# terryye/cuda_FlashAttention

Measured on AMD Instinct MI355X. Metric: FA2 fwd+bwd TFLOP/s at (B=4,H=16,N=8192,d=128); % MFMA peak, higher is better.
Workload: dtype bf16; 1 GPU; FA2 forward+backward bf16, (B=4,H=16,N=8192,d=128) per GPU, non-causal (BASELINE configs[2]); flops = 14 B H N^2 d; B=4, H=16, N=8192, d=128, parallelism=head-sharded replicas x1

## Files before the change

### cuda_flashattention_amd/csrc/fa2_bwd_fused.hip

```cpp
#include <cstdlib>
#include <cstring>
#include <type_traits>

#include "fa2_common.h"
#include "fa2_launch.h"

namespace fa2 {

#include "fa2_bwd_fused_body.inc"

typedef __attribute__((address_space(3))) void* fused_lptr_t;

#ifndef FA2_FUSED_DSKEY
#define FA2_FUSED_DSKEY(row) (((row) >> 1) & 7)
#endif

#ifndef FA2_FUSED_DIAG
#define FA2_FUSED_DIAG 0
#endif

template <int R>
__device__ __forceinline__ void fused_vset(uint32_t x)
{
    asm volatile("v_mov_b32 v%c1, %0" : : "v"(x), "i"(R) : "v255");
}

#define FA2_FUSED_CLOBBERS "memory", "vcc", "v255", FA2_ACC_CLOBBERS
#define FA2_FUSED_OPS [r0] "v"(roff[0]), [r1] "v"(roff[1]), [r2] "v"(roff[2]), [r3] "v"(roff[3]), [r4] "v"(roff[4]), [r5] "v"(roff[5]),  \
    [r6] "v"(roff[6]), [r7] "v"(roff[7]), [t0] "v"(toff[0]), [t1] "v"(toff[1]), [t2] "v"(toff[2]), [t3] "v"(toff[3]), [t4] "v"(toff[4]),   \
    [t5] "v"(toff[5]), [t6] "v"(toff[6]), [t7] "v"(toff[7]), [rc] "v"(rcv), [c2] "s"(c2)

struct FusedStep {
    __amdgpu_buffer_rsrc_t drs, lrs, qrs, grs, rcrs, ctl;
    uint32_t dso, lso, qso, rcso, pvo, mso;
    int need, pval;
};
#define FA2_FUSED_OPS64 [r0] "v"(roff[0]), [r1] "v"(roff[1]), [r2] "v"(roff[2]), [r3] "v"(roff[3]), [t0] "v"(toff[0]), [t1] "v"(toff[1]),    \
    [t2] "v"(toff[2]), [t3] "v"(toff[3]), [rc] "v"(rcv), [c2] "s"(c2)
template <int BUF, int PAR, int VMW, bool MASKED>
__device__ __forceinline__ void fused_cbody(const uint32_t (&roff)[4], const uint32_t (&toff)[4], uint32_t rcv, float c2, uint32_t dqv,
                                            uint32_t dvo, uint32_t rcvo, uint32_t mw, uint32_t mw2, int wv, const FusedStep& f, int& err,
                                            int lo0 = 0, int lo1 = 0)
{
#define FA2_FUSED_CASE(B, P)                                                                                                          \
    if constexpr (BUF == B && PAR == P && MASKED)                                                                                     \
        asm volatile(FA2_FUSED64_MBODY_B##B##_P##P                                                                                    \
                     : [err] "+s"(err)                                                                                                \
                     : FA2_FUSED_OPS64, [vm] "i"(VMW), [dqv] "v"(dqv), [drs] "s"(f.drs), [dso] "s"(f.dso), [lrs] "s"(f.lrs), [lso] "s"(f.lso), \
                       [mw] "s"(mw), [mw2] "s"(mw2), [qrs] "s"(f.qrs), [grs] "s"(f.grs), [rcrs] "s"(f.rcrs), [qso] "s"(f.qso),           \
                       [rcso] "s"(f.rcso), [dvo] "v"(dvo), [rcvo] "v"(rcvo), [wv] "s"(wv), [ctl] "s"(f.ctl), [pvo] "s"(f.pvo),           \
                       [mso] "s"(f.mso), [need] "s"(f.need), [pval] "s"(f.pval), [lo0] "v"(lo0), [lo1] "v"(lo1)                        \
                     : FA2_FUSED_CLOBBERS, "s12", "s13", "scc", "exec", "m0", "v39");                                                 \
    if constexpr (BUF == B && PAR == P && !MASKED)                                                                                    \
        asm volatile(FA2_FUSED64_CBODY_B##B##_P##P                                                                                    \
                     : [err] "+s"(err)                                                                                                \
                     : FA2_FUSED_OPS64, [vm] "i"(VMW), [dqv] "v"(dqv), [drs] "s"(f.drs), [dso] "s"(f.dso), [lrs] "s"(f.lrs), [lso] "s"(f.lso), \
                       [mw] "s"(mw), [mw2] "s"(mw2), [qrs] "s"(f.qrs), [grs] "s"(f.grs), [rcrs] "s"(f.rcrs), [qso] "s"(f.qso),           \
                       [rcso] "s"(f.rcso), [dvo] "v"(dvo), [rcvo] "v"(rcvo), [wv] "s"(wv), [ctl] "s"(f.ctl), [pvo] "s"(f.pvo),           \
                       [mso] "s"(f.mso), [need] "s"(f.need), [pval] "s"(f.pval)                                                        \
                     : FA2_FUSED_CLOBBERS, "s12", "s13", "scc", "exec", "m0", "v39");
    FA2_FUSED_CASE(0, 0) FA2_FUSED_CASE(0, 1) FA2_FUSED_CASE(1, 0) FA2_FUSED_CASE(1, 1) FA2_FUSED_CASE(2, 0) FA2_FUSED_CASE(2, 1)
#undef FA2_FUSED_CASE
}

template <int BUF, int PAR, int VMW, bool MASKED>
__device__ __forceinline__ void fused_cbody(const uint32_t (&roff)[8], const uint32_t (&toff)[8], uint32_t rcv, float c2, uint32_t dqv,
                                            uint32_t dvo, uint32_t rcvo, uint32_t mw, uint32_t mw2, int wv, const FusedStep& f, int& err,
                                            int lo0 = 0, int lo1 = 0)
{
#define FA2_FUSED_CASE(B, P)                                                                                                          \
    if constexpr (BUF == B && PAR == P && MASKED)                                                                                     \
        asm volatile(FA2_FUSED_MBODY_B##B##_P##P                                                                                      \
                     : [err] "+s"(err)                                                                                                \
                     : FA2_FUSED_OPS, [vm] "i"(VMW), [dqv] "v"(dqv), [drs] "s"(f.drs), [dso] "s"(f.dso), [lrs] "s"(f.lrs), [lso] "s"(f.lso), \
                       [mw] "s"(mw), [mw2] "s"(mw2), [qrs] "s"(f.qrs), [grs] "s"(f.grs), [rcrs] "s"(f.rcrs), [qso] "s"(f.qso),           \
                       [rcso] "s"(f.rcso), [dvo] "v"(dvo), [rcvo] "v"(rcvo), [wv] "s"(wv), [ctl] "s"(f.ctl), [pvo] "s"(f.pvo),           \
                       [mso] "s"(f.mso), [need] "s"(f.need), [pval] "s"(f.pval), [lo0] "v"(lo0), [lo1] "v"(lo1)                        \
                     : FA2_FUSED_CLOBBERS, "s12", "s13", "scc", "exec", "m0", "v39");                                                 \
    if constexpr (BUF == B && PAR == P && !MASKED)                                                                                    \
        asm volatile(FA2_FUSED_CBODY_B##B##_P##P                                                                                      \
                     : [err] "+s"(err)                                                                                                \
                     : FA2_FUSED_OPS, [vm] "i"(VMW), [dqv] "v"(dqv), [drs] "s"(f.drs), [dso] "s"(f.dso), [lrs] "s"(f.lrs), [lso] "s"(f.lso), \
                       [mw] "s"(mw), [mw2] "s"(mw2), [qrs] "s"(f.qrs), [grs] "s"(f.grs), [rcrs] "s"(f.rcrs), [qso] "s"(f.qso),           \
                       [rcso] "s"(f.rcso), [dvo] "v"(dvo), [rcvo] "v"(rcvo), [wv] "s"(wv), [ctl] "s"(f.ctl), [pvo] "s"(f.pvo),           \
                       [mso] "s"(f.mso), [need] "s"(f.need), [pval] "s"(f.pval)                                                        \
                     : FA2_FUSED_CLOBBERS, "s12", "s13", "scc", "exec", "m0", "v39");
    FA2_FUSED_CASE(0, 0) FA2_FUSED_CASE(0, 1) FA2_FUSED_CASE(1, 0) FA2_FUSED_CASE(1, 1) FA2_FUSED_CASE(2, 0) FA2_FUSED_CASE(2, 1)
#undef FA2_FUSED_CASE
}

template <int BUF, int PAR, int VMW>
__device__ __forceinline__ void fused_body(const uint32_t (&roff)[8], const uint32_t (&toff)[8], uint32_t rcv, float c2)
{
#define FA2_FUSED_CASE(B, P) \
    if constexpr (BUF == B && PAR == P) asm volatile(FA2_FUSED_BODY_B##B##_P##P : : FA2_FUSED_OPS, [vm] "i"(VMW) : FA2_FUSED_CLOBBERS);
    FA2_FUSED_CASE(0, 0) FA2_FUSED_CASE(0, 1) FA2_FUSED_CASE(1, 0) FA2_FUSED_CASE(1, 1) FA2_FUSED_CASE(2, 0) FA2_FUSED_CASE(2, 1)
#undef FA2_FUSED_CASE
}

template <int DQT>
__device__ __forceinline__ void fused_dq_atomic(__amdgpu_buffer_rsrc_t rs, uint32_t voff, uint32_t soff)
{
    asm volatile(
        "s_add_u32 s12, %2, 4096\n\ts_add_u32 s13, %2, 8192\n\ts_add_u32 s14, %2, 12288\n\t"
        "buffer_atomic_add_f32 v%c3, %0, %1, %2 offen\n\tbuffer_atomic_add_f32 v%c4, %0, %1, %2 offen offset:512\n\t"
        "buffer_atomic_add_f32 v%c5, %0, %1, %2 offen offset:1024\n\tbuffer_atomic_add_f32 v%c6, %0, %1, %2 offen offset:1536\n\t"
        "buffer_atomic_add_f32 v%c7, %0, %1, s12 offen\n\tbuffer_atomic_add_f32 v%c8, %0, %1, s12 offen offset:512\n\t"
        "buffer_atomic_add_f32 v%c9, %0, %1, s12 offen offset:1024\n\tbuffer_atomic_add_f32 v%c10, %0, %1, s12 offen offset:1536\n\t"
        "buffer_atomic_add_f32 v%c11, %0, %1, s13 offen\n\tbuffer_atomic_add_f32 v%c12, %0, %1, s13 offen offset:512\n\t"
        "buffer_atomic_add_f32 v%c13, %0, %1, s13 offen offset:1024\n\tbuffer_atomic_add_f32 v%c14, %0, %1, s13 offen offset:1536\n\t"
        "buffer_atomic_add_f32 v%c15, %0, %1, s14 offen\n\tbuffer_atomic_add_f32 v%c16, %0, %1, s14 offen offset:512\n\t"
        "buffer_atomic_add_f32 v%c17, %0, %1, s14 offen offset:1024\n\tbuffer_atomic_add_f32 v%c18, %0, %1, s14 offen offset:1536\n\t"
        "s_nop 1"
        : : "v"(voff), "s"(rs), "s"(soff), "i"(DQT), "i"(DQT + 1), "i"(DQT + 2), "i"(DQT + 3), "i"(DQT + 4), "i"(DQT + 5), "i"(DQT + 6),
            "i"(DQT + 7), "i"(DQT + 8), "i"(DQT + 9), "i"(DQT + 10), "i"(DQT + 11), "i"(DQT + 12), "i"(DQT + 13), "i"(DQT + 14),
            "i"(DQT + 15)
        : "memory", "s12", "s13", "s14", "v255");
}

template <int VF, int KS, int S>
__device__ __forceinline__ void fused_load_vfrag(const char* v0, const char* v1)
{
#ifndef FA2_FUSED_KV_NT
#define FA2_FUSED_KV_NT ""
#define FA2_FUSED_KV_AUX 0
#endif
    asm volatile("global_load_dwordx4 v[%c2:%c3], %0, off offset:%c4" FA2_FUSED_KV_NT "\n\tglobal_load_dwordx4 v[%c5:%c6], %1, off offset:%c4" FA2_FUSED_KV_NT
                 : : "v"(v0), "v"(v1), "i"(VF + 4 * S), "i"(VF + 4 * S + 3), "i"(32 * S), "i"(VF + 4 * (KS + S)), "i"(VF + 4 * (KS + S) + 3)
                 : "memory", "v255");
}

template <int T>
__device__ __forceinline__ void fused_acc_zero(u32x4 z)
{
    asm volatile("s_nop 1\n\tv_mfma_f32_32x32x16_bf16 a[%c1:%c2], %0, %0, 0" : : "v"(z), "i"(16 * T), "i"(16 * T + 15) : FA2_ACC_CLOBBERS);
}

template <int DQT>
__device__ __forceinline__ void fused_dq_zero()
{
    static_for<16>([&](auto R) { fused_vset<DQT + decltype(R)::value>(0u); });
}

constexpr int kCtlTicket = 0, kCtlNextHead = 32 * 16, kCtlError = 32 * 17, kCtlHeadmap = 32 * 18;
constexpr int kHmPad = 16;
constexpr int kSpinLimit = FA2_FUSED_SPIN_LIMIT;

struct FusedArgs {
    BwdArgs b;
    float* dQacc;
    int* ctl;
    int npad;
    const float* rc;
    int fault;
};

#ifdef FA2_TEST_HOOKS
static int g_hook_fault = 0, g_hook_grid = 0, g_hook_last_grid = 0;
extern "C" void fa2_test_set_fused_hooks(int fault, int grid) { g_hook_fault = fault; g_hook_grid = grid; }
extern "C" int fa2_test_last_fused_grid(void) { return g_hook_last_grid; }
#define FA2_HOOK_NOTE_GRID(n) (g_hook_last_grid = (n))
#else
constexpr int g_hook_fault = 0, g_hook_grid = 0;
#define FA2_HOOK_NOTE_GRID(n) ((void)0)
#endif

__device__ __forceinline__ int fused_ctl_ints(int BH, int ncb) { return kCtlHeadmap + 16 * (BH + kHmPad) + 9 * BH * ncb; }

__device__ __forceinline__ int fused_load_sc1(const int* p)
{
    int v;
    asm volatile("global_load_dword %0, %1, off sc1\n\ts_waitcnt vmcnt(0)" : "=v"(v) : "v"(p) : "memory");
    return v;
}
__device__ __forceinline__ void fused_seen_set(int v)
{
    asm volatile("v_mov_b32 v39, %0" : : "s"(v) : "v39");
}

__device__ __forceinline__ int fused_lane_id() { return (int)__builtin_amdgcn_mbcnt_hi(~0u, __builtin_amdgcn_mbcnt_lo(~0u, 0u)); }
template <int OFF>
__device__ __forceinline__ int fused_mail_read(uint32_t lds_addr)
{
    int v;
    asm volatile("v_mov_b32 %0, %1\n\tds_read_b32 %0, %0 offset:%c2\n\ts_waitcnt lgkmcnt(0)" : "=&v"(v) : "s"(lds_addr), "i"(OFF) : "memory");
    return __builtin_amdgcn_readfirstlane(v);
}

__device__ __forceinline__ void fused_store_flag(int* p, int v)
{
    asm volatile("global_store_dword %0, %1, off" : : "v"(p), "v"(v) : "memory");
}

__device__ __forceinline__ bool fused_spin_over(int* ctl, int spins)
{
    if (spins > kSpinLimit) {
        atomicExch(ctl + kCtlError, 1);
        return true;
    }
    return (spins & 1023) == 0 && fused_load_sc1(ctl + kCtlError) != 0;
}

template <bool CHAIN, bool CAUSAL, bool RAGGED = false, bool RECT = false, int HD = 128>
__global__ void __launch_bounds__(256, 1) __attribute__((amdgpu_num_vgpr(39))) fa2_bwd_fused_kernel(FusedArgs fp)
{
    static_assert(CHAIN || !RAGGED, "the atomics form has no ragged variant");
    static_assert(!RECT || (CHAIN && !CAUSAL && !RAGGED), "rectangular blocks: chained, unmasked, aligned");
    static_assert(HD == 128 || (HD == 64 && CHAIN && !RECT), "head_dim 64: chained, square");
    extern __shared__ __attribute__((aligned(16))) char smem[];
    const BwdArgs& p = fp.b;
    constexpr int D = HD, ROWB = 2 * D, KS = D / 16, DT = D / 32;
    constexpr int DQW = 128;
    constexpr int TROWS = 32;
    constexpr bool W = D == 128;
    constexpr int QRING = W ? FA2_FUSED_QRING : FA2_FUSED64_QRING, BUFB = W ? FA2_FUSED_BUFB : FA2_FUSED64_BUFB,
                  DSB = W ? FA2_FUSED_DSB : FA2_FUSED64_DSB, LDSB = W ? FA2_FUSED_LDS : FA2_FUSED64_LDS;
    constexpr int CPR = D / 8, RPI = 64 / CPR, NINS = TROWS / RPI;
    constexpr int VF = W ? FA2_FUSED_VF : FA2_FUSED64_VF, DQT = W ? FA2_FUSED_DQT : FA2_FUSED64_DQT,
                  ROFFK = W ? FA2_FUSED_ROFFK : FA2_FUSED64_ROFFK, DSWR = W ? FA2_FUSED_DSWR : FA2_FUSED64_DSWR,
                  DSRD = W ? FA2_FUSED_DSRD : FA2_FUSED64_DSRD, KT = W ? FA2_FUSED_KT : FA2_FUSED64_KT;
    constexpr int VMW = CHAIN ? (W ? 4 : 2) : 63;
    int* const mail = reinterpret_cast<int*>(smem + LDSB);
    const uint32_t mail_addr = __builtin_amdgcn_readfirstlane((uint32_t)(uintptr_t)smem) + LDSB;

    const int tid = threadIdx.x;
    const int lane = tid & 63;
    const int wave = __builtin_amdgcn_readfirstlane(tid >> 6);
    const int ki = lane & 31;
    const int h = lane >> 5;
    const int N = p.Nk;
    const int NP = RAGGED ? fp.npad : N;
    const int NQ = RECT ? p.Nq : N;
    const int NPQ = RECT ? NQ : NP;
    const int QHS = RECT ? p.q_hs : N, KHS = RECT ? p.k_hs : N;
    const int QR0 = RECT ? p.q_row0 : 0;
    const int ncb = NP / 256;
    const int ntiles = NPQ / TROWS;
    const int niter = ((ntiles + 1 + 5) / 6) * 6;
    const float c2 = p.scale * kLog2e;
    const size_t rc_plane = (size_t)p.BH * (RECT ? QHS : NP);

    const uint32_t lbase = (uint32_t)(uintptr_t)smem;
    const int trq = (lane & 15) >> 2, trp = lane & 3, trcb = (lane >> 4) & 1;
    uint32_t roff[KS], toff[2 * DT];
#pragma unroll
    for (int s = 0; s < KS; ++s) roff[s] = lbase + QRING + lds_off<D>(ki, 2 * s + h);
#pragma unroll
    for (int dt = 0; dt < DT; ++dt)
#pragma unroll
        for (int jj = 0; jj < 2; ++jj)
            toff[2 * dt + jj] = lbase + QRING + lds_off<D>(8 * jj + 4 * h + trq, 4 * dt + 2 * trcb + (trp >> 1)) + 8 * (trp & 1);
    const uint32_t rcv = lbase + QRING + 2 * TROWS * ROWB + 16 * h;
    static_for<KS>([&](auto S) {
        constexpr int sidx = decltype(S)::value;
        fused_vset<ROFFK + sidx>(lbase + lds_off<D>(ki + 64 * wave, 2 * sidx + h));
    });
    const int ecol = W ? wave : (wave & 1), ekey0 = W ? 0 : 128 * (wave >> 1);
    static_for<2>([&](auto JJ) {
        constexpr int jj = decltype(JJ)::value;
        fused_vset<KT + jj>(lbase + ekey0 * ROWB + lds_off<D>(8 * jj + 4 * h + trq, 4 * ecol + 2 * trcb + (trp >> 1)) + 8 * (trp & 1));
        const int row = 8 * jj + 4 * h + trq;
        fused_vset<DSRD + jj>(lbase + DSB + (ekey0 + row) * 64 + 8 * ((4 * trcb + trp) ^ FA2_FUSED_DSKEY(row)));
    });
    static_for<4>([&](auto C) {
        constexpr int c = decltype(C)::value;
        fused_vset<DSWR + c>(lbase + DSB + (64 * wave + ki) * 64 + 8 * (((2 * c) | h) ^ FA2_FUSED_DSKEY(ki)));
    });
    const int drow = lane / CPR, dslot = lane % CPR;
    const int prow = wave * RPI + drow;
    const int doff = drow * ROWB + 16 * ((lds_off<D>(prow, dslot) - ROWB * prow) >> 4);
    const uint32_t dqv = CHAIN ? (uint32_t)(wave * 4096 + lane * 16) : (uint32_t)(((4 * h) * D + 32 * wave + ki) * 4);
    const auto rc_rsrc = __builtin_amdgcn_make_buffer_rsrc((void*)fp.rc, 0, (int)(2 * rc_plane * 4), 0x00020000);

    int xcc = 0;
    if constexpr (CHAIN) {
        asm volatile("s_getreg_b32 %0, hwreg(HW_REG_XCC_ID, 0, 4)" : "=s"(xcc));
    }
    int* const prog_base = fp.ctl + kCtlHeadmap + 16 * (p.BH + kHmPad);
#ifndef FA2_FUSED_CAUSAL_G
#define FA2_FUSED_CAUSAL_G 2
#endif
    const int G = CAUSAL ? max(1, min(FA2_FUSED_CAUSAL_G, p.BH / 8)) : 1;
    const auto ctl_rsrc = __builtin_amdgcn_make_buffer_rsrc((void*)fp.ctl, 0, CHAIN ? fused_ctl_ints(p.BH, ncb) * 4 : 0, 0x00020000);

    auto take_ticket = [&]() {
        if (wave == 0 && fused_lane_id() == 0) {
            int hd, j = 0;
            do {
                const int u = atomicAdd(fp.ctl + kCtlTicket + 32 * xcc, 1);
                const int r = u % (G * ncb);
                const int k = (u / (G * ncb)) * G + r % G;
                j = r / G;
                hd = -2;
                if (k < p.BH + kHmPad) {
                    int* hm = fp.ctl + kCtlHeadmap + xcc * (p.BH + kHmPad) + k;
                    int v = 0, spins = 0;
                    if (j == 0) {
                        if (k > 0)
                            while ((v = fused_load_sc1(hm - 1)) == 0)
                                if (fused_spin_over(fp.ctl, ++spins)) break;
                        if (k > 0 && v == 0) {
                            v = -1;
                        } else {
                            const int g = atomicAdd(fp.ctl + kCtlNextHead, 1);
                            v = g < p.BH ? g + 1 : -1;
                        }
                        fused_store_flag(hm, v);
                    } else {
                        while ((v = fused_load_sc1(hm)) == 0)
                            if (fused_spin_over(fp.ctl, ++spins)) { v = -1; break; }
                    }
                    hd = v > 0 ? v - 1 : (r % G == 0 ? -2 : -1);
                }
            } while (hd == -1);
            mail[0] = hd;
            mail[1] = j;
            mail[2] = hd >= 0 ? fused_load_sc1(fp.ctl + kCtlError) : 0;
        }
    };
    auto issue_unit_loads = [&](int head_, int cb_) {
        const size_t slab_ = (size_t)(head_ / p.kv_group) * KHS * ROWB;
        const char* Kh_ = (const char*)p.K + slab_;
        const char* Vh_ = (const char*)p.V + slab_;
        const int kw0_ = cb_ * 256 + wave * 64;
        const int lane_u = (int)__builtin_amdgcn_mbcnt_hi(~0u, __builtin_amdgcn_mbcnt_lo(~0u, 0u));
        const int vk0 = RAGGED ? min(kw0_ + (lane_u & 31), N - 1) : kw0_ + (lane_u & 31);
        const int vk1 = RAGGED ? min(kw0_ + 32 + (lane_u & 31), N - 1) : kw0_ + 32 + (lane_u & 31);
        const char* v0 = Vh_ + (size_t)vk0 * ROWB + 16 * (lane_u >> 5);
        const char* v1 = Vh_ + (size_t)vk1 * ROWB + 16 * (lane_u >> 5);
        static_for<KS>([&](auto S) { fused_load_vfrag<VF, KS, decltype(S)::value>(v0, v1); });
        const auto k_rsrc = __builtin_amdgcn_make_buffer_rsrc((void*)Kh_, 0, N * ROWB, 0x00020000);
#pragma unroll
        for (int j = wave; j < 256 / RPI; j += 4)
            __builtin_amdgcn_raw_ptr_buffer_load_lds(k_rsrc, (fused_lptr_t)(smem + j * 1024), 16, doff, (cb_ * 256 + j * RPI) * ROWB, 0, FA2_FUSED_KV_AUX);
    };

    auto next_unit_loads = [&]() {
        if constexpr (CHAIN) {
            take_ticket();
            __syncthreads();
            const int hn = fused_mail_read<0>(mail_addr);
            if (hn >= 0) issue_unit_loads(hn, fused_mail_read<4>(mail_addr));
        }
    };
    next_unit_loads();

    for (;;) {
#ifdef FA2_FUSED_STATS
        const uint64_t s_pull = __builtin_readcyclecounter();
#endif
        int head, cb, err0 = 0;
        if constexpr (CHAIN) {
            head = fused_mail_read<0>(mail_addr);
            cb = fused_mail_read<4>(mail_addr);
            err0 = fused_mail_read<8>(mail_addr);
            if (head < 0) break;
        } else {
            map_block(blockIdx.x, p.BH, ncb, head, cb);
            issue_unit_loads(head, cb);
        }
        const size_t slab = (size_t)head * QHS * ROWB;
        const char* Qh = (const char*)p.Q + slab;
        const char* Gh = (const char*)p.dO + slab;
        const int kw0 = cb * 256 + wave * 64;
        {
            const u32x4 z = {0u, 0u, 0u, 0u};
            static_for<4 * DT>([&](auto T) { fused_acc_zero<decltype(T)::value>(z); });
        }

        const auto q_rsrc = __builtin_amdgcn_make_buffer_rsrc((void*)Qh, 0, NQ * ROWB, 0x00020000);
        const auto g_rsrc = __builtin_amdgcn_make_buffer_rsrc((void*)Gh, 0, NQ * ROWB, 0x00020000);
        const int rcoff = (int)(((wave == 0 ? 0 : rc_plane) + (size_t)head * (RECT ? QHS : NP) + QR0 + (fused_lane_id() & 31)) * 4);
        auto stage = [&](int t, int buf) {
            char* b = smem + QRING + buf * BUFB;
#pragma unroll
            for (int j = wave; j < 2 * NINS; j += 4) {
                const int which = j / NINS, piece = j % NINS;
                const int soff = (t * TROWS + piece * RPI) * ROWB;
                __builtin_amdgcn_raw_ptr_buffer_load_lds(which ? g_rsrc : q_rsrc, (fused_lptr_t)(b + which * (TROWS * ROWB) + piece * 1024),
                                                         16, doff, soff, 0, 0);
            }
            if (wave < 2 && fused_lane_id() < 32)
                __builtin_amdgcn_raw_ptr_buffer_load_lds(rc_rsrc, (fused_lptr_t)(b + 2 * TROWS * ROWB + wave * 128), 4, rcoff, t * TROWS * 4, 0, 0);
        };
        const int n_u = CAUSAL ? ntiles - 8 * cb : ntiles;
        const int niter_u = CAUSAL ? ((n_u + 1 + 5) / 6) * 6 : niter;
        const bool ragged_unit = RAGGED && !CAUSAL && cb == ncb - 1;
        const int first_masked = CAUSAL ? ((n_u - 8) / 6) * 6 : (ragged_unit ? 0 : niter_u);
        auto tl = [&](int u) { return CAUSAL ? ntiles - 1 - u : u; };
        stage(tl(0), 0);
#ifdef FA2_FUSED_PREFILL
        stage(tl(1), 1);
        stage(tl(2), 2);
#endif
        fused_dq_zero<DQT>();
        asm volatile("s_waitcnt vmcnt(0)" ::: "memory");
        __syncthreads();
        if constexpr (W) asm volatile(FA2_FUSED_PRO : : FA2_FUSED_OPS, [vm] "i"(VMW) : FA2_FUSED_CLOBBERS);
        else asm volatile(FA2_FUSED64_PRO : : FA2_FUSED_OPS64, [vm] "i"(VMW) : FA2_FUSED_CLOBBERS);

        const auto dq_rsrc = __builtin_amdgcn_make_buffer_rsrc((void*)(fp.dQacc + (size_t)head * NPQ * DQW), 0, NPQ * DQW * 4, 0x00020000);
        int* const mine = prog_base + head * ncb + cb;
        const int* const prev = mine - 1;
        const int prev_off = (int)((prev - fp.ctl) * 4);
        const int mine_off = (int)((mine - fp.ctl) * 4);
        if constexpr (CHAIN) fused_seen_set(0);
        int err = err0;
#ifdef FA2_FUSED_STATS
        int st_steps = 0, st_polls = 0, st_cycles = 0;
        const uint64_t u0 = __builtin_readcyclecounter();
#endif

        const auto null_rsrc = __builtin_amdgcn_make_buffer_rsrc((void*)fp.dQacc, 0, 0, 0x00020000);
        const bool hp_unit = cb > 0;
        const auto lrs_unit = hp_unit && !(FA2_FUSED_DIAG & 2) ? dq_rsrc : null_rsrc;
        auto step = [&](auto BUF, auto PAR, auto MASKED, auto FAST_, int t) {
            constexpr int buf = decltype(BUF)::value, par = decltype(PAR)::value;
            constexpr bool masked = decltype(MASKED)::value;
            constexpr bool FAST = decltype(FAST_)::value;
            if constexpr (CHAIN && FAST) {
                FusedStep f;
                f.drs = dq_rsrc;
                f.lrs = lrs_unit;
                f.dso = (uint32_t)(tl(t - 1) * TROWS * DQW * 4);
                f.lso = (uint32_t)(tl(t) * TROWS * DQW * 4);
                f.qrs = q_rsrc; f.grs = g_rsrc; f.rcrs = rc_rsrc; f.ctl = ctl_rsrc;
                f.qso = (uint32_t)(tl(t + 1) * TROWS * ROWB + wave * 1024);
                f.rcso = (uint32_t)(tl(t + 1) * TROWS * 4);
                f.pvo = (uint32_t)prev_off; f.mso = (uint32_t)mine_off;
                f.need = (hp_unit && !err && !(FA2_FUSED_DIAG & 1)) ? t + 1 : (int)0x80000000;
                f.pval = t;
#ifdef FA2_TEST_HOOKS
                if (fp.fault && cb == 1) f.pval = 0;
#endif
                fused_cbody<buf, par, VMW, false>(roff, toff, rcv, c2, dqv, (uint32_t)doff, (uint32_t)rcoff, lbase + QRING + wave * 1024,
                                                  lbase + QRING + wave * 128, wave, f, err, 0, 0);
            } else if constexpr (CHAIN) {
                FusedStep f;
                const bool live = t >= 1 && t <= n_u;
                const bool more = t + 1 < n_u;
                const bool has_prev = t < n_u && cb > 0;
                f.drs = live ? dq_rsrc : null_rsrc;
                f.lrs = has_prev && !(FA2_FUSED_DIAG & 2) ? dq_rsrc : null_rsrc;
                f.dso = (uint32_t)__builtin_amdgcn_readfirstlane(tl(t - 1) * TROWS * DQW * 4);
                f.lso = (uint32_t)__builtin_amdgcn_readfirstlane(tl(t) * TROWS * DQW * 4);
                f.qrs = q_rsrc; f.grs = g_rsrc; f.rcrs = rc_rsrc; f.ctl = ctl_rsrc;
                f.qso = more ? (uint32_t)(tl(t + 1) * TROWS * ROWB + wave * 1024) : 0x40000000u;
                f.rcso = more ? (uint32_t)(tl(t + 1) * TROWS * 4) : 0x40000000u;
                f.pvo = (uint32_t)prev_off; f.mso = (uint32_t)mine_off;
                f.need = (has_prev && !err && !(FA2_FUSED_DIAG & 1)) ? t + 1 : (int)0x80000000;
                f.pval = t < n_u ? t : n_u;
#ifdef FA2_TEST_HOOKS
                if (fp.fault && cb == 1) f.pval = 0;
#endif
                int lo0 = 0, lo1 = 0;
                if constexpr (masked) {
                    const int lane_m = (int)__builtin_amdgcn_mbcnt_hi(~0u, __builtin_amdgcn_mbcnt_lo(~0u, 0u));
                    if constexpr (CAUSAL) {
                        lo0 = kw0 + (lane_m & 31) - 4 * (lane_m >> 5) - TROWS * tl(t);
                        lo1 = lo0 + 32;
                    } else {
                        lo0 = kw0 + (lane_m & 31) < N ? -0x40000000 : 0x40000000;
                        lo1 = kw0 + 32 + (lane_m & 31) < N ? -0x40000000 : 0x40000000;
                    }
                }
#ifdef FA2_FUSED_STATS2
                const uint64_t b0 = __builtin_readcyclecounter();
#endif
                fused_cbody<buf, par, VMW, masked>(roff, toff, rcv, c2, dqv, (uint32_t)doff, (uint32_t)rcoff, lbase + QRING + wave * 1024,
                                                   lbase + QRING + wave * 128, wave, f, err, lo0, lo1);
#ifdef FA2_FUSED_STATS2
                st_cycles += (int)(__builtin_readcyclecounter() - b0);
#endif
            } else {
                static_assert(W || CHAIN, "head_dim 64: chained form only");
                stage(t + 1, (buf + 1) % 3);
                if constexpr (W) fused_body<buf, par, VMW>(roff, toff, rcv, c2);
#ifndef FA2_FUSED_NO_DQ
                if (t >= 1 && t <= ntiles) fused_dq_atomic<DQT>(dq_rsrc, dqv, (uint32_t)__builtin_amdgcn_readfirstlane((t - 1) * TROWS * D * 4));
#endif
                fused_dq_zero<DQT>();
            }
        };
        auto six = [&](auto MASKED, auto FAST_, int t) {
            step(std::integral_constant<int, 0>{}, std::integral_constant<int, 0>{}, MASKED, FAST_, t);
            step(std::integral_constant<int, 1>{}, std::integral_constant<int, 1>{}, MASKED, FAST_, t + 1);
            step(std::integral_constant<int, 2>{}, std::integral_constant<int, 0>{}, MASKED, FAST_, t + 2);
            step(std::integral_constant<int, 0>{}, std::integral_constant<int, 1>{}, MASKED, FAST_, t + 3);
            step(std::integral_constant<int, 1>{}, std::integral_constant<int, 0>{}, MASKED, FAST_, t + 4);
            step(std::integral_constant<int, 2>{}, std::integral_constant<int, 1>{}, MASKED, FAST_, t + 5);
        };
        const int fast_end = CHAIN ? n_u - 2 : -1;
        {
            const int plain_end = first_masked;
            int t = 0;
            asm volatile("" : "+s"(t));
            if (t < plain_end) { six(std::false_type{}, std::false_type{}, t); t += 6; }
#pragma unroll 1
            for (; t + 5 <= fast_end && t < plain_end; t += 6) six(std::false_type{}, std::true_type{}, t);
#pragma unroll 1
            for (; t < plain_end; t += 6) six(std::false_type{}, std::false_type{}, t);
            if constexpr (CHAIN && (CAUSAL || RAGGED)) {
#pragma unroll 1
                for (; t < niter_u; t += 6) six(std::true_type{}, std::false_type{}, t);
            }
        }
        asm volatile("s_waitcnt vmcnt(0) lgkmcnt(0)" ::: "memory");
        if constexpr (CHAIN)
            if (err && !err0 && wave == 0 && fused_lane_id() == 0) atomicExch(fp.ctl + kCtlError, 1);
#ifdef FA2_FUSED_STATS
        const uint64_t s_loop = __builtin_readcyclecounter();
#endif
        next_unit_loads();

        mfma_acc_settle();
        const int lane_ep = (int)__builtin_amdgcn_mbcnt_hi(~0u, __builtin_amdgcn_mbcnt_lo(~0u, 0u));
        const int ki_ep = lane_ep & 31, h_ep = lane_ep >> 5;
        static_for<2>([&](auto KB) {
            constexpr int kb = decltype(KB)::value;
            const int key = kw0 + 32 * kb + ki_ep;
            const size_t slab_k = RECT ? (size_t)head * KHS * ROWB : slab;
            char* const dKb = (char*)p.dK + slab_k;
            char* const dVb = (char*)p.dV + slab_k;
            const uint32_t koff = (uint32_t)key * ROWB + 16u * h_ep;
            char* dKk = dKb + koff;
            char* dVk = dVb + koff;
            static_for<2 * DT>([&](auto G) {
                constexpr int dt = decltype(G)::value / 2, gp = decltype(G)::value % 2;
                constexpr int RK = 16 * (kb * DT + dt) + 8 * gp, RV = 32 * DT + RK;
                auto pack4 = [&](float a, float b, float c, float d, float sc) {
                    bf16x4 v;
                    v[0] = (__bf16)(a * sc); v[1] = (__bf16)(b * sc); v[2] = (__bf16)(c * sc); v[3] = (__bf16)(d * sc);
                    return __builtin_bit_cast(u32x2, v);
                };
                auto emit = [&](u32x2 x, u32x2 y, char* dst) {
                    const auto s0 = __builtin_amdgcn_permlane32_swap(x[0], y[0], false, false);
                    const auto s1 = __builtin_amdgcn_permlane32_swap(x[1], y[1], false, false);
                    const u32x4 o = {s0[0], s1[0], s0[1], s1[1]};
#ifdef FA2_FUSED_ST_NT
                    if (!RAGGED || key < N) __builtin_nontemporal_store(o, reinterpret_cast<u32x4*>(dst + 2 * (32 * dt + 16 * gp)));
#else
                    if (!RAGGED || key < N) *reinterpret_cast<u32x4*>(dst + 2 * (32 * dt + 16 * gp)) = o;
#endif
                };
                emit(pack4(acc_read<RK>(), acc_read<RK + 1>(), acc_read<RK + 2>(), acc_read<RK + 3>(), p.scale),
                     pack4(acc_read<RK + 4>(), acc_read<RK + 5>(), acc_read<RK + 6>(), acc_read<RK + 7>(), p.scale), dKk);
                emit(pack4(acc_read<RV>(), acc_read<RV + 1>(), acc_read<RV + 2>(), acc_read<RV + 3>(), 1.0f),
                     pack4(acc_read<RV + 4>(), acc_read<RV + 5>(), acc_read<RV + 6>(), acc_read<RV + 7>(), 1.0f), dVk);
            });
        });
#ifdef FA2_FUSED_STATS
        if (CHAIN && wave == 0 && fused_lane_id() == 0) {
            atomicAdd(fp.ctl + kCtlError + 1, st_steps);
            atomicAdd(fp.ctl + kCtlError + 2, st_polls);
            atomicAdd((unsigned long long*)(fp.ctl + kCtlError + 4), (unsigned long long)st_cycles);
            atomicAdd((unsigned long long*)(fp.ctl + kCtlError + 6), (unsigned long long)(__builtin_readcyclecounter() - u0));
            int* rec = prog_base + p.BH * ncb + 8 * (head * ncb + cb);
            rec[0] = xcc; rec[1] = st_cycles; rec[2] = (int)(u0 - s_pull); rec[3] = (int)(__builtin_readcyclecounter() - s_loop);
            *(unsigned long long*)(rec + 4) = u0; *(unsigned long long*)(rec + 6) = __builtin_readcyclecounter();
        }
#endif
        if constexpr (!CHAIN) break;
    }
}

__global__ void __launch_bounds__(256) fa2_bwd_fused_dq_out_kernel(const float* __restrict__ acc, __bf16* __restrict__ dQ, size_t n8, float scale,
                                                                    const int* __restrict__ err)
{
    const float poison = (err && *err) ? __builtin_nanf("") : 0.0f;
    const size_t stride = (size_t)gridDim.x * 256;
    for (size_t i = (size_t)blockIdx.x * 256 + threadIdx.x; i < n8; i += stride) {
        const f32x4 a = reinterpret_cast<const f32x4*>(acc)[2 * i], b = reinterpret_cast<const f32x4*>(acc)[2 * i + 1];
        bf16x8 o;
#pragma unroll
        for (int e = 0; e < 4; ++e) { o[e] = (__bf16)(a[e] * scale + poison); o[4 + e] = (__bf16)(b[e] * scale + poison); }
        reinterpret_cast<bf16x8*>(dQ)[i] = o;
    }
}

__global__ void __launch_bounds__(256) fa2_bwd_fused_dq_out_chain_kernel(const float* __restrict__ acc, __bf16* __restrict__ dQ, size_t n4, float scale,
                                                                          const int* __restrict__ err, int N, int NP, int qhs)
{
    const float poison = *err ? __builtin_nanf("") : 0.0f;
    const size_t stride = (size_t)gridDim.x * 256;
    const size_t tiles = (size_t)(NP / 32);
    for (size_t i = (size_t)blockIdx.x * 256 + threadIdx.x; i < n4; i += stride) {
        const f32x4 a = reinterpret_cast<const f32x4*>(acc)[i];
        const int lane = (int)(i & 63), g = (int)((i >> 6) & 3), wave = (int)((i >> 8) & 3);
        const size_t tg = i >> 10, head = tg / tiles;
        const int row = (int)(tg % tiles) * 32 + 8 * g + 4 * (lane >> 5);
        __bf16* o = dQ + (head * (size_t)qhs + row) * 128 + 32 * wave + (lane & 31);
#pragma unroll
        for (int e = 0; e < 4; ++e)
            if (row + e < N) o[(size_t)e * 128] = (__bf16)(a[e] * scale + poison);
    }
}

__global__ void __launch_bounds__(256) fa2_bwd_fused_dq_out_chain64_kernel(const float* __restrict__ acc, __bf16* __restrict__ dQ, size_t n4h, float scale,
                                                                            const int* __restrict__ err, int N, int NP)
{
    const float poison = *err ? __builtin_nanf("") : 0.0f;
    const size_t stride = (size_t)gridDim.x * 256;
    const size_t tiles = (size_t)(NP / 32);
    for (size_t i = (size_t)blockIdx.x * 256 + threadIdx.x; i < n4h; i += stride) {
        const int lane = (int)(i & 63), g = (int)((i >> 6) & 3), cbk = (int)((i >> 8) & 1);
        const size_t tg = i >> 9, head = tg / tiles;
        const size_t slot = ((tg * 4 + cbk) * 4 + g) * 64 + lane;
        const f32x4 a = reinterpret_cast<const f32x4*>(acc)[slot], b = reinterpret_cast<const f32x4*>(acc)[slot + 2 * 4 * 64];
        const int row = (int)(tg % tiles) * 32 + 8 * g + 4 * (lane >> 5);
        __bf16* o = dQ + (head * (size_t)N + row) * 64 + 32 * cbk + (lane & 31);
#pragma unroll
        for (int e = 0; e < 4; ++e)
            if (row + e < N) o[(size_t)e * 64] = (__bf16)((a[e] + b[e]) * scale + poison);
    }
}

__global__ void __launch_bounds__(256) fa2_bwd_fused_dkdv_out_kernel(const bf16x8* __restrict__ pK, const bf16x8* __restrict__ pV,
                                                                      bf16x8* __restrict__ dK, bf16x8* __restrict__ dV, size_t n8, size_t nkv, int G)
{
    const size_t stride = (size_t)gridDim.x * 256;
    for (size_t i = (size_t)blockIdx.x * 256 + threadIdx.x; i < 2 * nkv * n8; i += stride) {
        const bool isv = i >= nkv * n8;
        const size_t o = isv ? i - nkv * n8 : i, kvh = o / n8, r = o % n8;
        const bf16x8* src = (isv ? pV : pK) + kvh * (size_t)G * n8 + r;
        float s[8] = {};
        for (int g = 0; g < G; ++g) {
            const bf16x8 x = src[(size_t)g * n8];
#pragma unroll
            for (int e = 0; e < 8; ++e) s[e] += (float)x[e];
        }
        bf16x8 out;
#pragma unroll
        for (int e = 0; e < 8; ++e) out[e] = (__bf16)s[e];
        (isv ? dV : dK)[o] = out;
    }
}

__global__ void __launch_bounds__(256) fa2_bwd_fused_rcpad_kernel(const float* __restrict__ rc, float* __restrict__ out, int BH, int N, int NP)
{
    const size_t per = (size_t)BH * NP, i = (size_t)blockIdx.x * 256 + threadIdx.x;
    if (i >= 2 * per) return;
    const size_t plane = i / per, r = i % per, head = r / NP;
    const int row = (int)(r % NP);
    out[i] = row < N ? rc[plane * (size_t)BH * N + head * (size_t)N + row] : (plane == 0 ? -1.0e30f : 0.0f);
}

bool bwd_fused_device_ok(const char** why)
{
    static int verdict[64] = {};
    int dev = 0;
    if (hipGetDevice(&dev) != hipSuccess || dev < 0 || dev >= 64) { if (why) *why = "no current device"; return false; }
    if (!verdict[dev]) {
        hipDeviceProp_t pr;
        if (hipGetDeviceProperties(&pr, dev) != hipSuccess) { if (why) *why = "device properties unavailable"; return false; }
        verdict[dev] = strncmp(pr.gcnArchName, "gfx950", 6) != 0 ? 2 : pr.multiProcessorCount != 256 ? 3 : 1;
    }
    static const char* const text[] = {"", "single five-product kernel (gfx950, 256 CUs: the layout the ordered hand-off was validated on)",
                                       "two kernels: device is not gfx950", "two kernels: device does not expose 256 CUs (partitioned GPU): "
                                       "the ordered hand-off was validated in SPX mode only"};
    if (why) *why = text[verdict[dev]];
    return verdict[dev] == 1;
}

hipError_t bwd_fused_read_error(const int* ctl, int* err, hipStream_t stream)
{
    hipError_t e = hipMemcpyAsync(err, ctl + kCtlError, sizeof(int), hipMemcpyDeviceToHost, stream);
    if (e != hipSuccess) return e;
    return hipStreamSynchronize(stream);
}

hipError_t bwd_fused_clear_error(int* ctl, hipStream_t stream)
{
    return launch_fill_f32(reinterpret_cast<float*>(ctl + kCtlError), 1, 0.0f, stream);
}

size_t bwd_fused_kvpart_bytes(int BH, int N, int d) { return (size_t)2 * BH * N * d * 2; }
size_t bwd_fused_ctl_bytes(int BH, int N) { return (size_t)(kCtlHeadmap + 16 * (BH + kHmPad) + 9 * BH * ((N + 255) / 256)) * sizeof(int); }

template <int HD>
static hipError_t launch_chained_square(bool causal, bool ragged, dim3 grid, int lds, hipStream_t stream, const FusedArgs& fa)
{
    if (causal)
        return ragged ? launch_lds<fa2_bwd_fused_kernel<true, true, true, false, HD>>(grid, dim3(256), lds, stream, fa)
                      : launch_lds<fa2_bwd_fused_kernel<true, true, false, false, HD>>(grid, dim3(256), lds, stream, fa);
    return ragged ? launch_lds<fa2_bwd_fused_kernel<true, false, true, false, HD>>(grid, dim3(256), lds, stream, fa)
                  : launch_lds<fa2_bwd_fused_kernel<true, false, false, false, HD>>(grid, dim3(256), lds, stream, fa);
}

hipError_t launch_bwd_fused_bf16(const BwdArgs& a, float* dQacc, int* ctl, int mode, hipStream_t stream, float* rcpad, void* kvpart)
{
    const int npad = (a.Nk + 255) / 256 * 256;
    const bool ragged = npad != a.Nk;
    const bool rect = a.Nq != a.Nk || a.q_hs != a.Nq || a.k_hs != a.Nk || a.q_row0 != 0;
    if ((a.d != 128 && a.d != 64) || a.Nk < 1 || a.Nq < 1) return hipErrorInvalidValue;
    if (a.d == 64 && (mode != 1 || rect)) return hipErrorInvalidValue;
    if (rect && (mode != 1 || a.causal || ragged || a.Nq % 32 != 0 || a.q_row0 < 0 || a.q_hs < a.q_row0 + a.Nq || a.k_hs < a.Nk))
        return hipErrorInvalidValue;
    if (ragged && (mode != 1 || !rcpad)) return hipErrorInvalidValue;
    const bool grouped = a.kv_group > 1;
    if (a.kv_group < 1 || a.BH % a.kv_group != 0 || (grouped && (mode != 1 || rect || !kvpart))) return hipErrorInvalidValue;
    if (a.causal && (mode != 1 || a.causal_shift != 0)) return hipErrorInvalidValue;
    hipError_t e = hipSuccess;
    if (a.phases & 1) {
        BwdArgs d = a;
        d.phases = 1;
        e = launch_bwd_bf16(d, stream);
        if (e != hipSuccess) return e;
    }
    if (!(a.phases & 8)) return hipSuccess;
    const size_t elems = (size_t)a.BH * (rect ? a.Nq : npad) * 128;
    const int units = a.BH * (npad / 256);
    if (ragged) {
        const size_t n = (size_t)2 * a.BH * npad;
        hipLaunchKernelGGL(fa2_bwd_fused_rcpad_kernel, dim3((unsigned)((n + 255) / 256)), dim3(256), 0, stream, (const float*)a.RC, rcpad,
                           a.BH, a.Nk, npad);
        e = hipGetLastError();
        if (e != hipSuccess) return e;
    }
    FusedArgs fa{a, dQacc, ctl, npad, ragged ? (const float*)rcpad : (const float*)a.RC, g_hook_fault};
    const size_t part_elems = (size_t)a.BH * a.Nk * a.d;
    if (grouped) {
        fa.b.dK = kvpart;
        fa.b.dV = (__bf16*)kvpart + part_elems;
    }
    const int lds = (a.d == 64 ? FA2_FUSED64_LDS : FA2_FUSED_LDS) + 16;
    if (mode == 0) {
        e = launch_fill_f32(dQacc, elems, 0.0f, stream);
        if (e != hipSuccess) return e;
        e = bwd_fused_clear_error(ctl, stream);
        if (e != hipSuccess) return e;
        e = launch_lds<fa2_bwd_fused_kernel<false, false>>(dim3((unsigned)units), dim3(256), lds, stream, fa);
    } else {
        static int cus[64] = {};
        int dev = 0;
        e = hipGetDevice(&dev);
        if (e != hipSuccess) return e;
        if (dev < 0 || dev >= 64) return hipErrorInvalidDevice;
        if (!cus[dev]) {
            e = hipDeviceGetAttribute(&cus[dev], hipDeviceAttributeMultiprocessorCount, dev);
            if (e != hipSuccess) return e;
        }
        e = launch_fill_f32(reinterpret_cast<float*>(ctl), bwd_fused_ctl_bytes(a.BH, a.Nk) / sizeof(float), 0.0f, stream);
        if (e != hipSuccess) return e;
        int avail = cus[dev] - (a.reserve_cus > 0 ? a.reserve_cus : 0);
        if (avail < 1) avail = 1;
        int wgs = units < avail ? units : avail;
        if (g_hook_grid >= 1 && g_hook_grid < wgs) wgs = g_hook_grid;
        FA2_HOOK_NOTE_GRID(wgs);
        const dim3 grid((unsigned)wgs);
        if (rect)
            e = launch_lds<fa2_bwd_fused_kernel<true, false, false, true>>(grid, dim3(256), lds, stream, fa);
        else
            e = a.d == 64 ? launch_chained_square<64>(a.causal, ragged, grid, lds, stream, fa)
                          : launch_chained_square<128>(a.causal, ragged, grid, lds, stream, fa);
    }
    if (e != hipSuccess) return e;
    if (mode == 0)
        hipLaunchKernelGGL(fa2_bwd_fused_dq_out_kernel, dim3(2048), dim3(256), 0, stream, dQacc, (__bf16*)a.dQ, elems / 8, a.scale,
                           (const int*)nullptr);
    else if (a.d == 64)
        hipLaunchKernelGGL(fa2_bwd_fused_dq_out_chain64_kernel, dim3(4096), dim3(256), 0, stream, dQacc, (__bf16*)a.dQ, elems / 8, a.scale,
                           ctl + kCtlError, a.Nk, npad);
    else
        hipLaunchKernelGGL(fa2_bwd_fused_dq_out_chain_kernel, dim3(4096), dim3(256), 0, stream, dQacc, (__bf16*)a.dQ, elems / 4, a.scale,
                           ctl + kCtlError, rect ? a.Nq : a.Nk, rect ? a.Nq : npad, rect ? a.q_hs : a.Nk);
    e = hipGetLastError();
    if (e != hipSuccess || !grouped) return e;
    hipLaunchKernelGGL(fa2_bwd_fused_dkdv_out_kernel, dim3(4096), dim3(256), 0, stream, (const bf16x8*)fa.b.dK, (const bf16x8*)fa.b.dV,
                       (bf16x8*)a.dK, (bf16x8*)a.dV, (size_t)a.Nk * a.d / 8, (size_t)(a.BH / a.kv_group), a.kv_group);
    return hipGetLastError();
}

}
```

Before: 1325 TFLOP/s.

## Fuse dQ fp32-to-bf16 conversion into chained fused backward kernel

In the persistent chained backward kernel, workgroups that pick up a ticket for the next head also convert the finished dQ accumulator pieces of the previous head from fp32 to bf16. A piece is converted once that head's progress counter shows it is done. This replaces the separate dQ output kernel with a light guard kernel that only writes NaNs when the error flag is set. The aim is to remove an extra full pass over the fp32 dQ buffer and its kernel launch, in exchange for extra spinning and inline-asm work inside the main kernel and some added scheduling complexity.

```diff
diff --git a/cuda_flashattention_amd/csrc/fa2_bwd_fused.hip b/cuda_flashattention_amd/csrc/fa2_bwd_fused.hip
--- a/cuda_flashattention_amd/csrc/fa2_bwd_fused.hip
+++ b/cuda_flashattention_amd/csrc/fa2_bwd_fused.hip
@@ -153,16 +153,22 @@
     int npad;
     const float* rc;
     int fault;
+    int conv;
 };
 
 #ifdef FA2_TEST_HOOKS
-static int g_hook_fault = 0, g_hook_grid = 0, g_hook_last_grid = 0;
+static int g_hook_fault = 0, g_hook_grid = 0, g_hook_last_grid = 0, g_hook_dq_pass = 0;
+static const int* g_hook_last_ctl = nullptr;
+static int g_hook_last_bh = 0, g_hook_last_ncb = 0;
 extern "C" void fa2_test_set_fused_hooks(int fault, int grid) { g_hook_fault = fault; g_hook_grid = grid; }
 extern "C" int fa2_test_last_fused_grid(void) { return g_hook_last_grid; }
+extern "C" void fa2_test_set_fused_dq_pass(int on) { g_hook_dq_pass = on; }
 #define FA2_HOOK_NOTE_GRID(n) (g_hook_last_grid = (n))
+#define FA2_HOOK_NOTE_CTL(c, bh, ncb) (g_hook_last_ctl = (c), g_hook_last_bh = (bh), g_hook_last_ncb = (ncb))
 #else
-constexpr int g_hook_fault = 0, g_hook_grid = 0;
+constexpr int g_hook_fault = 0, g_hook_grid = 0, g_hook_dq_pass = 0;
 #define FA2_HOOK_NOTE_GRID(n) ((void)0)
+#define FA2_HOOK_NOTE_CTL(c, bh, ncb) ((void)0)
 #endif
 
 __device__ __forceinline__ int fused_ctl_ints(int BH, int ncb) { return kCtlHeadmap + 16 * (BH + kHmPad) + 9 * BH * ncb; }
@@ -173,6 +179,62 @@
     asm volatile("global_load_dword %0, %1, off sc1\n\ts_waitcnt vmcnt(0)" : "=v"(v) : "v"(p) : "memory");
     return v;
 }
+__device__ __forceinline__ void fused_load2_sc1(const int* p, int& before, int& at)
+{
+    asm volatile("global_load_dword %0, %2, off offset:-4 sc1\n\tglobal_load_dword %1, %2, off sc1\n\ts_waitcnt vmcnt(0)"
+                 : "=&v"(before), "=&v"(at) : "v"(p) : "memory");
+}
+
+#define FA2_CV_A(s, e) "v[104+4*(" #s ")+" #e "]"
+#define FA2_CV_Q(s) "v[104+4*(" #s "):107+4*(" #s ")]"
+#define FA2_CV_T(s, e) "v[168+2*(" #s ")+" #e "]"
+#define FA2_CV_TP(s) "v[168+2*(" #s "):169+2*(" #s ")]"
+#define FA2_CV_DPP(perm) " quad_perm:[" perm "] row_mask:0xf bank_mask:0xf\n\t"
+#define FA2_CV_LOAD(w, g) "buffer_load_dwordx4 " FA2_CV_Q(4*w+g) ", v201, %[irs], s[12+" #w "] offen offset:1024*" #g " sc1\n\t"
+#define FA2_CV_STORE(w, g) "buffer_store_dwordx2 " FA2_CV_TP(4*w+g) ", v202, %[ors], s[12+" #g "/2] offen offset:2048*(" #g "%%2)+64*" #w "\n\t"
+#define FA2_CV_FMA(s)                                                                                                                 \
+    "v_fma_f32 " FA2_CV_A(s, 0) ", " FA2_CV_A(s, 0) ", %[sc], v204\n\tv_fma_f32 " FA2_CV_A(s, 1) ", " FA2_CV_A(s, 1) ", %[sc], v204\n\t" \
+    "v_fma_f32 " FA2_CV_A(s, 2) ", " FA2_CV_A(s, 2) ", %[sc], v204\n\tv_fma_f32 " FA2_CV_A(s, 3) ", " FA2_CV_A(s, 3) ", %[sc], v204\n\t"
+#define FA2_CV_X1(s)                                                                                                                  \
+    "v_cndmask_b32_dpp " FA2_CV_T(s, 0) ", " FA2_CV_A(s, 1) ", " FA2_CV_A(s, 0) ", vcc" FA2_CV_DPP("1,0,3,2")                            \
+    "v_cndmask_b32_dpp " FA2_CV_T(s, 1) ", " FA2_CV_A(s, 3) ", " FA2_CV_A(s, 2) ", vcc" FA2_CV_DPP("1,0,3,2")
+#define FA2_CV_X2(s)                                                                                                                  \
+    "v_cndmask_b32_dpp " FA2_CV_A(s, 1) ", " FA2_CV_A(s, 0) ", " FA2_CV_A(s, 1) ", vcc" FA2_CV_DPP("1,0,3,2")                            \
+    "v_cndmask_b32_dpp " FA2_CV_A(s, 3) ", " FA2_CV_A(s, 2) ", " FA2_CV_A(s, 3) ", vcc" FA2_CV_DPP("1,0,3,2")
+#define FA2_CV_PK(s)                                                                                                                  \
+    "v_cvt_pk_bf16_f32 " FA2_CV_A(s, 0) ", " FA2_CV_T(s, 0) ", " FA2_CV_A(s, 1) "\n\t"                                                  \
+    "v_cvt_pk_bf16_f32 " FA2_CV_A(s, 2) ", " FA2_CV_T(s, 1) ", " FA2_CV_A(s, 3) "\n\t"
+#define FA2_CV_X3(s) "v_cndmask_b32_dpp " FA2_CV_T(s, 0) ", " FA2_CV_A(s, 2) ", " FA2_CV_A(s, 0) ", vcc" FA2_CV_DPP("2,3,0,1")
+#define FA2_CV_X4(s) "v_cndmask_b32_dpp " FA2_CV_T(s, 1) ", " FA2_CV_A(s, 0) ", " FA2_CV_A(s, 2) ", vcc" FA2_CV_DPP("2,3,0,1")
+#define FA2_CV_ALL(M) M(0) M(1) M(2) M(3) M(4) M(5) M(6) M(7) M(8) M(9) M(10) M(11) M(12) M(13) M(14) M(15)
+#define FA2_CV_ALL2(M) M(0, 0) M(0, 1) M(0, 2) M(0, 3) M(1, 0) M(1, 1) M(1, 2) M(1, 3) M(2, 0) M(2, 1) M(2, 2) M(2, 3) M(3, 0) M(3, 1) M(3, 2) M(3, 3)
+#define FA2_CV_VCC(m) "s_mov_b32 vcc_lo, " m "\n\ts_mov_b32 vcc_hi, " m "\n\ts_nop 1\n\t"
+__device__ __forceinline__ void fused_convert_round(__amdgpu_buffer_rsrc_t irs, uint32_t iso, __amdgpu_buffer_rsrc_t ors, uint32_t oso,
+                                                    float scale, float poison)
+{
+    asm volatile(
+        "v_mbcnt_lo_u32_b32 v200, -1, 0\n\tv_mbcnt_hi_u32_b32 v200, -1, v200\n\t"
+        "v_lshlrev_b32 v201, 4, v200\n\t"
+        "v_lshrrev_b32 v202, 5, v200\n\tv_and_b32 v203, 3, v200\n\tv_lshl_add_u32 v202, v202, 2, v203\n\t"
+        "v_lshlrev_b32 v202, 8, v202\n\tv_bfe_u32 v203, v200, 2, 3\n\tv_lshl_add_u32 v202, v203, 3, v202\n\t"
+        "v_mov_b32 v204, %[po]\n\t"
+        "s_add_u32 s12, %[iso], 0\n\ts_add_u32 s13, %[iso], 4096\n\ts_add_u32 s14, %[iso], 8192\n\ts_add_u32 s15, %[iso], 12288\n\t"
+        FA2_CV_ALL2(FA2_CV_LOAD)
+        "s_waitcnt vmcnt(0)\n\t"
+        FA2_CV_ALL(FA2_CV_FMA)
+        FA2_CV_VCC("0x55555555") FA2_CV_ALL(FA2_CV_X1)
+        FA2_CV_VCC("0xaaaaaaaa") FA2_CV_ALL(FA2_CV_X2)
+        "s_nop 1\n\t"
+        FA2_CV_ALL(FA2_CV_PK)
+        FA2_CV_VCC("0x33333333") FA2_CV_ALL(FA2_CV_X3)
+        FA2_CV_VCC("0xcccccccc") FA2_CV_ALL(FA2_CV_X4)
+        "s_add_u32 s12, %[oso], 0\n\ts_add_u32 s13, %[oso], 4096\n\ts_nop 1\n\t"
+        FA2_CV_ALL2(FA2_CV_STORE)
+        "s_nop 0"
+        : : [irs] "s"(irs), [iso] "s"(iso), [ors] "s"(ors), [oso] "s"(oso), [sc] "s"(scale), [po] "s"(poison)
+        : "memory", "vcc", "scc", "s12", "s13", "s14", "s15", "v255");
+}
+
 __device__ __forceinline__ void fused_seen_set(int v)
 {
     asm volatile("v_mov_b32 v39, %0" : : "s"(v) : "v39");
@@ -285,21 +347,23 @@
 
     auto take_ticket = [&]() {
         if (wave == 0 && fused_lane_id() == 0) {
-            int hd, j = 0;
+            int hd, j = 0, cv;
             do {
                 const int u = atomicAdd(fp.ctl + kCtlTicket + 32 * xcc, 1);
                 const int r = u % (G * ncb);
                 const int k = (u / (G * ncb)) * G + r % G;
                 j = r / G;
                 hd = -2;
+                cv = -1;
                 if (k < p.BH + kHmPad) {
                     int* hm = fp.ctl + kCtlHeadmap + xcc * (p.BH + kHmPad) + k;
-                    int v = 0, spins = 0;
+                    int v = 0, vp = 0, spins = 0;
                     if (j == 0) {
                         if (k > 0)
                             while ((v = fused_load_sc1(hm - 1)) == 0)
                                 if (fused_spin_over(fp.ctl, ++spins)) break;
-                        if (k > 0 && v == 0) {
+                        vp = v;
+                        if (k > 0 && v <= 0) {
                             v = -1;
                         } else {
                             const int g = atomicAdd(fp.ctl + kCtlNextHead, 1);
@@ -307,15 +371,24 @@
                         }
                         fused_store_flag(hm, v);
                     } else {
-                        while ((v = fused_load_sc1(hm)) == 0)
+                        for (;;) {
+                            fused_load2_sc1(hm, vp, v);
+                            if (v != 0) break;
                             if (fused_spin_over(fp.ctl, ++spins)) { v = -1; break; }
+                        }
+                        if (fp.conv && k > 0 && vp == 0) vp = fused_load_sc1(hm - 1);
                     }
                     hd = v > 0 ? v - 1 : (r % G == 0 ? -2 : -1);
+                    if (fp.conv && k > 0 && vp > 0) {
+                        cv = vp - 1;
+                        if (hd < 0) hd = -1;
+                    }
                 }
-            } while (hd == -1);
+            } while (hd == -1 && cv < 0);
             mail[0] = hd;
             mail[1] = j;
-            mail[2] = hd >= 0 ? fused_load_sc1(fp.ctl + kCtlError) : 0;
+            mail[2] = (hd >= 0 || cv >= 0) ? fused_load_sc1(fp.ctl + kCtlError) : 0;
+            mail[3] = cv;
         }
     };
     auto issue_unit_loads = [&](int head_, int cb_) {
@@ -343,7 +416,43 @@
             if (hn >= 0) issue_unit_loads(hn, fused_mail_read<4>(mail_addr));
         }
     };
+    constexpr bool CONVERTS = CHAIN && !CAUSAL && !RAGGED && !RECT && HD == 128;
+    auto convert_piece = [&](int cvh, int cb_, int errw) {
+        const int* pw = prog_base + cvh * ncb + (ncb - 1);
+        int bad = errw;
+        if (!bad && !(FA2_FUSED_DIAG & 1)) {
+            int spins = 0;
+            while (__builtin_amdgcn_readfirstlane(fused_load_sc1(pw)) < 8 * cb_ + 8)
+                if (__builtin_amdgcn_readfirstlane((int)fused_spin_over(fp.ctl, ++spins))) { bad = 1; break; }
+        }
+        const float poison = bad ? __builtin_nanf("") : 0.0f;
+        const auto in_rsrc = __builtin_amdgcn_make_buffer_rsrc((void*)(fp.dQacc + (size_t)cvh * NP * DQW), 0, NP * DQW * 4, 0x00020000);
+        const auto out_rsrc = __builtin_amdgcn_make_buffer_rsrc((void*)((char*)p.dQ + (size_t)cvh * N * ROWB), 0, N * ROWB, 0x00020000);
+#pragma unroll 1
+        for (int r = 0; r < 2; ++r) {
+            const int tile = 8 * cb_ + 2 * wave + r;
+            fused_convert_round(in_rsrc, (uint32_t)(tile * TROWS * DQW * 4), out_rsrc, (uint32_t)(tile * TROWS * ROWB), p.scale, poison);
+        }
+#ifdef FA2_TEST_HOOKS
+        if (wave == 0 && fused_lane_id() == 0) fused_store_flag(prog_base + p.BH * ncb + 8 * (cvh * ncb + cb_), (int)blockIdx.x + 1);
+#endif
+    };
+    auto convert_pending = [&]() {
+        if constexpr (CONVERTS) {
+            if (fp.conv) {
+                for (;;) {
+                    const int cvh = fused_mail_read<12>(mail_addr);
+                    const int hn = fused_mail_read<0>(mail_addr);
+                    if (cvh >= 0) convert_piece(cvh, fused_mail_read<4>(mail_addr), fused_mail_read<8>(mail_addr));
+                    if (hn != -1) break;
+                    __syncthreads();
+                    next_unit_loads();
+                }
+            }
+        }
+    };
     next_unit_loads();
+    convert_pending();
 
     for (;;) {
 #ifdef FA2_FUSED_STATS
@@ -549,6 +658,7 @@
                      pack4(acc_read<RV + 4>(), acc_read<RV + 5>(), acc_read<RV + 6>(), acc_read<RV + 7>(), 1.0f), dVk);
             });
         });
+        convert_pending();
 #ifdef FA2_FUSED_STATS
         if (CHAIN && wave == 0 && fused_lane_id() == 0) {
             atomicAdd(fp.ctl + kCtlError + 1, st_steps);
@@ -594,6 +704,14 @@
         for (int e = 0; e < 4; ++e)
             if (row + e < N) o[(size_t)e * 128] = (__bf16)(a[e] * scale + poison);
     }
+}
+
+__global__ void __launch_bounds__(256) fa2_bwd_fused_dq_guard_kernel(const int* __restrict__ err, u32x4* __restrict__ dQ, size_t n8)
+{
+    if (*err == 0) return;
+    const u32x4 nan8 = {0x7fc07fc0u, 0x7fc07fc0u, 0x7fc07fc0u, 0x7fc07fc0u};
+    const size_t stride = (size_t)gridDim.x * 256;
+    for (size_t i = (size_t)blockIdx.x * 256 + threadIdx.x; i < n8; i += stride) dQ[i] = nan8;
 }
 
 __global__ void __launch_bounds__(256) fa2_bwd_fused_dq_out_chain64_kernel(const float* __restrict__ acc, __bf16* __restrict__ dQ, size_t n4h, float scale,
@@ -676,6 +794,17 @@
 
 size_t bwd_fused_kvpart_bytes(int BH, int N, int d) { return (size_t)2 * BH * N * d * 2; }
 size_t bwd_fused_ctl_bytes(int BH, int N) { return (size_t)(kCtlHeadmap + 16 * (BH + kHmPad) + 9 * BH * ((N + 255) / 256)) * sizeof(int); }
+
+#ifdef FA2_TEST_HOOKS
+extern "C" int fa2_test_fused_conv_owners(int* out, int n)
+{
+    const int pieces = g_hook_last_bh * g_hook_last_ncb;
+    if (!g_hook_last_ctl || n < pieces) return -1;
+    const int* rec = g_hook_last_ctl + kCtlHeadmap + 16 * (g_hook_last_bh + kHmPad) + pieces;
+    if (hipMemcpy2D(out, sizeof(int), rec, 8 * sizeof(int), sizeof(int), (size_t)pieces, hipMemcpyDeviceToHost) != hipSuccess) return -1;
+    return pieces;
+}
+#endif
 
 template <int HD>
 static hipError_t launch_chained_square(bool causal, bool ragged, dim3 grid, int lds, hipStream_t stream, const FusedArgs& fa)
@@ -717,7 +846,8 @@
         e = hipGetLastError();
         if (e != hipSuccess) return e;
     }
-    FusedArgs fa{a, dQacc, ctl, npad, ragged ? (const float*)rcpad : (const float*)a.RC, g_hook_fault};
+    const bool conv = mode == 1 && a.d == 128 && !a.causal && !ragged && !rect && !g_hook_dq_pass;
+    FusedArgs fa{a, dQacc, ctl, npad, ragged ? (const float*)rcpad : (const float*)a.RC, g_hook_fault, conv ? 1 : 0};
     const size_t part_elems = (size_t)a.BH * a.Nk * a.d;
     if (grouped) {
         fa.b.dK = kvpart;
@@ -747,6 +877,7 @@
         int wgs = units < avail ? units : avail;
         if (g_hook_grid >= 1 && g_hook_grid < wgs) wgs = g_hook_grid;
         FA2_HOOK_NOTE_GRID(wgs);
+        FA2_HOOK_NOTE_CTL(ctl, a.BH, npad / 256);
         const dim3 grid((unsigned)wgs);
         if (rect)
             e = launch_lds<fa2_bwd_fused_kernel<true, false, false, true>>(grid, dim3(256), lds, stream, fa);
@@ -758,6 +889,8 @@
     if (mode == 0)
         hipLaunchKernelGGL(fa2_bwd_fused_dq_out_kernel, dim3(2048), dim3(256), 0, stream, dQacc, (__bf16*)a.dQ, elems / 8, a.scale,
                            (const int*)nullptr);
+    else if (conv)
+        hipLaunchKernelGGL(fa2_bwd_fused_dq_guard_kernel, dim3(256), dim3(256), 0, stream, (const int*)(ctl + kCtlError), (u32x4*)a.dQ, elems / 8);
     else if (a.d == 64)
         hipLaunchKernelGGL(fa2_bwd_fused_dq_out_chain64_kernel, dim3(4096), dim3(256), 0, stream, dQacc, (__bf16*)a.dQ, elems / 8, a.scale,
                            ctl + kCtlError, a.Nk, npad);
```

Measured after the change: 1332 TFLOP/s, median of 6. Within noise of the previous version (+0.5%).
